# Linux-cpp-lisp/sitator

Measured on AMD Instinct MI355X. Metric: landmark-vectors/sec (frames x mobile atoms), fill + site assignment, higher is better.
Workload: dtype f64; 1 GPU; C2: SCgrid(8,8,8) orthorhombic 32.0x35.2x38.4 A, S=D=512 (V=8), M=64, A=576 (BASELINE configs[1]), 100000 frames per GPU; frames_per_gpu=100000, n_mobile=64, n_static=512, landmark_dim=512, parallelism=frame-sharded x1

## Files before the change

### sitator_amd/csrc/cluster.hip

```cpp
#include <cmath>
#include <cstring>
#include <hip/amd_detail/amd_hip_unsafe_atomics.h>

#include <algorithm>

#include "sit_internal.h"

__device__ __forceinline__ Best wave_best(Best b)
{
    for (int off = 32; off > 0; off >>= 1) {
        Best o;
        o.v = __shfl_down(b.v, off);
        o.i = __shfl_down(b.i, off);
        o.nan = __shfl_down(b.nan, off);
        b = best_merge(b, o);
    }
    return b;
}

#define PRED_BLOCK 256
#define PRED_MAXCOL 24

struct PredArgs {
    const i32 *row_nnz, *row_idx;
    const double *row_val;
    const i32 *col_ptr, *col_k;
    const double *col_val;
    const double *dense;
    i64 *labels;
    double *confs;
    i64 N, K, D;
    int normed;
    double threshold;
};

__device__ __forceinline__ i64 finish_predict(const PredArgs &a, i64 row, Best b)
{
    i64 to; double conf;
    finish_assignment(b, a.threshold, to, conf);
    __builtin_nontemporal_store(to, &a.labels[row]);
    __builtin_nontemporal_store(conf, &a.confs[row]);
    return to;
}

__device__ i64 predict_row_generic(const PredArgs &a, i64 row, int n, double xn)
{
    Best b = best_empty();
    for (int e = 0; e < n; e++) {
        const i32 d = a.row_idx[(i64)e * a.N + row];
        const i32 lo = a.col_ptr[d], hi = a.col_ptr[d + 1];
        for (i32 q = lo; q < hi; q++) {
            const i32 cid = a.col_k[q];
            const double *crow = a.dense + (i64)cid * a.D;
            bool owner = true;
            for (int e2 = 0; e2 < e; e2++) {
                const double cv = crow[a.row_idx[(i64)e2 * a.N + row]];
                if (cv != 0.0) { owner = false; break; }
            }
            if (!owner) continue;
            double dot = 0.0;
            bool first = true;
            for (int e3 = e; e3 < n; e3++) {
                const double cv = crow[a.row_idx[(i64)e3 * a.N + row]];
                if (cv != 0.0) {
                    const double t = cv * a.row_val[(i64)e3 * a.N + row];
                    dot = first ? t : dot + t;
                    first = false;
                }
            }
            if (a.normed) dot /= xn;
            b = best_merge(b, best_of(fabs(dot), cid));
        }
    }
    return finish_predict(a, row, b);
}

__device__ __forceinline__ i64 predict_row_merge(const PredArgs &a, i64 row, int n, double xn)
{
    i32 d0 = a.row_idx[row], d1 = 0, d2 = 0, d3 = 0;
    double v0 = a.row_val[row], v1 = 0, v2 = 0, v3 = 0;
    if (n > 1) { d1 = a.row_idx[a.N + row]; v1 = a.row_val[a.N + row]; }
    if (n > 2) { d2 = a.row_idx[2 * a.N + row]; v2 = a.row_val[2 * a.N + row]; }
    if (n > 3) { d3 = a.row_idx[3 * a.N + row]; v3 = a.row_val[3 * a.N + row]; }
    return finish_predict(a, row, merge4_row(n, d0, d1, d2, d3, v0, v1, v2, v3, xn, a.normed != 0, a.col_ptr, a.col_k, a.col_val));
}

template <int NW>
__device__ __forceinline__ i64 predict_row_merge_wide(const PredArgs &a, i64 row, int n, double xn)
{
    ArgMaxQ am;
    am.init();
    const i32 none = 0x7fffffff;
    i32 q[NW], e[NW], h[NW];
    double v[NW];
#pragma unroll
    for (int s = 0; s < NW; s++) {
        q[s] = 0; e[s] = 0; h[s] = none; v[s] = 0.0;
        if (s < n) {
            const i32 d = a.row_idx[(i64)s * a.N + row];
            q[s] = a.col_ptr[d]; e[s] = a.col_ptr[d + 1]; v[s] = a.row_val[(i64)s * a.N + row];
            h[s] = q[s] < e[s] ? a.col_k[q[s]] : none;
        }
    }
    while (true) {
        i32 cid = h[0];
#pragma unroll
        for (int s = 1; s < NW; s++) cid = h[s] < cid ? h[s] : cid;
        if (cid == none) break;
        double dot = 0.0;
        bool first = true;
#pragma unroll
        for (int s = 0; s < NW; s++) {
            if (h[s] == cid) {
                const double t = a.col_val[q[s]] * v[s];
                dot = first ? t : dot + t;
                first = false;
                q[s]++;
                h[s] = q[s] < e[s] ? a.col_k[q[s]] : none;
            }
        }
        am.push(dot, cid, xn, a.normed != 0);
    }
    return finish_predict(a, row, am.result(xn, a.normed != 0));
}

__device__ __forceinline__ bool predict_row_head(const PredArgs &a, i64 row, int &n, double &xn)
{
    n = __builtin_nontemporal_load(&a.row_nnz[row]);
    if (n == 0) { __builtin_nontemporal_store((i64)-1, &a.labels[row]); __builtin_nontemporal_store(0.0, &a.confs[row]); return false; }
    double x2 = 0.0;
    for (int e = 0; e < n; e++) { const double v = a.row_val[(i64)e * a.N + row]; x2 += v * v; }
    xn = sqrt(x2);
    return true;
}

__device__ __forceinline__ void list_wide_rows(int n, bool live, i64 row, i32 *seg, unsigned *seg_count, i64 seg_cap, int lane)
{
    list_rows_by_class(live && n > 4 && n <= 8, live && n > 8, row, seg, seg_count, seg_cap, lane);
}

__global__ __launch_bounds__(PRED_BLOCK) void k_predict_rows(PredArgs a, i32 *wide_list, unsigned *wide_count, i64 seg_cap)
{
    i32 *seg = wide_list + (i64)blockIdx.x * seg_cap;
    unsigned *seg_count = wide_count + 2 * blockIdx.x;
    const int lane = threadIdx.x & 63;
    for (i64 r0 = (i64)blockIdx.x * PRED_BLOCK; r0 < a.N; r0 += (i64)gridDim.x * PRED_BLOCK) {
        const i64 row = r0 + threadIdx.x;
        int n = 0;
        double xn = 0.0;
        const bool live = row < a.N && predict_row_head(a, row, n, xn);
        const bool wide = live && n > 4;
        list_wide_rows(n, live, row, seg, seg_count, seg_cap, lane);
        if (live && !wide) predict_row_merge(a, row, n, xn);
    }
}

struct ArgMaxR {
    double ms;
    i32 i;
    __device__ __forceinline__ void init() { ms = 0.0; i = -1; }
    __device__ __forceinline__ void push(double dot, i32 cid, double xn, bool normed)
    {
        bool take = !(fabs(dot) <= fabs(ms));
        const bool clear = fabs(dot) > fabs(ms) * (1.0 + 1e-15);
        if (normed & take & !clear)
            take = dot != dot || fabs(dot) / xn > fabs(ms) / xn;
        take = take & (ms == ms);
        ms = take ? dot : ms;
        i = take ? cid : i;
    }
    __device__ __forceinline__ Best result(double xn, bool normed) const
    {
        Best b;
        const double m = fabs(ms);
        b.i = (i64)i; b.nan = m != m ? 1 : 0;
        b.v = i < 0 ? 0.0 : (normed ? m / xn : m);
        return b;
    }
};
typedef const unsigned __attribute__((address_space(3))) *LdsWords;
struct RecHead { i32 h; double hv; unsigned p; };
#define PRED_REC 12
__device__ __forceinline__ void rec_load(RecHead &c)
{
    LdsWords r = (LdsWords)(uintptr_t)c.p;
    const unsigned r0 = r[0], r1 = r[1], r2 = r[2];
    c.h = (i32)r2;
    c.hv = __hiloint2double((int)r1, (int)r0);
}
__device__ __forceinline__ Best merge4_rec(int n, i32 d0, i32 d1, i32 d2, i32 d3, double v0, double v1, double v2, double v3,
                                           double xn, bool normed, const unsigned *l_off)
{
    ArgMaxR am;
    am.init();
    const i32 none = 0x7fffffff;
    RecHead c0, c1, c2, c3;
    c0.p = l_off[d0]; rec_load(c0);
    c1.h = none; c1.hv = 0.0; c1.p = 0u;
    c2 = c1; c3 = c1;
    if (n > 1) { c1.p = l_off[d1]; rec_load(c1); }
    if (n > 2) { c2.p = l_off[d2]; rec_load(c2); }
    if (n > 3) { c3.p = l_off[d3]; rec_load(c3); }
    while (true) {
        i32 cid = c0.h < c1.h ? c0.h : c1.h;
        const i32 m23 = c2.h < c3.h ? c2.h : c3.h;
        cid = cid < m23 ? cid : m23;
        if (cid == none) break;
        double dot = 0.0;
        if (c0.h == cid) { dot = c0.hv * v0; c0.p += PRED_REC; rec_load(c0); }
        if (c1.h == cid) { dot = dot + c1.hv * v1; c1.p += PRED_REC; rec_load(c1); }
        if (c2.h == cid) { dot = dot + c2.hv * v2; c2.p += PRED_REC; rec_load(c2); }
        if (c3.h == cid) { dot = dot + c3.hv * v3; c3.p += PRED_REC; rec_load(c3); }
        am.push(dot, cid, xn, normed);
    }
    return am.result(xn, normed);
}

#define PRED_REC_BLOCK 1024
__global__ __launch_bounds__(PRED_REC_BLOCK) void k_predict_rows_rec(PredArgs a, const unsigned *recs, int nrec, i32 *wide_list, unsigned *wide_count,
                                                                     i64 seg_cap, int hist_K, u64 *counts)
{
    extern __shared__ __attribute__((aligned(16))) char pl_smem[];
    unsigned *l_rec = (unsigned *)pl_smem;
    unsigned *l_off = l_rec + 3 * nrec;
    unsigned *hist = l_off + a.D;
    const int NT = PRED_REC_BLOCK;
    for (int q = threadIdx.x; q < hist_K; q += NT) hist[q] = 0u;
    for (int q = threadIdx.x; q < 3 * nrec; q += NT) l_rec[q] = recs[q];
    for (int q = threadIdx.x; q < (int)a.D; q += NT) l_off[q] = (unsigned)(uintptr_t)(LdsWords)l_rec + (unsigned)PRED_REC * (unsigned)(a.col_ptr[q] + q);
    __syncthreads();
    i32 *seg = wide_list + (i64)blockIdx.x * seg_cap;
    unsigned *seg_count = wide_count + 2 * blockIdx.x;
    const int lane = threadIdx.x & 63;
    for (i64 r0 = (i64)blockIdx.x * NT; r0 < a.N; r0 += (i64)gridDim.x * NT) {
        const i64 row = r0 + threadIdx.x;
        int n = 0;
        double xn = 0.0;
        const bool live = row < a.N && predict_row_head(a, row, n, xn);
        const bool wide = live && n > 4;
        list_wide_rows(n, live, row, seg, seg_count, seg_cap, lane);
        if (live && !wide) {
            i32 d0 = a.row_idx[row], d1 = 0, d2 = 0, d3 = 0;
            double v0 = a.row_val[row], v1 = 0, v2 = 0, v3 = 0;
            if (n > 1) { d1 = a.row_idx[a.N + row]; v1 = a.row_val[a.N + row]; }
            if (n > 2) { d2 = a.row_idx[2 * a.N + row]; v2 = a.row_val[2 * a.N + row]; }
            if (n > 3) { d3 = a.row_idx[3 * a.N + row]; v3 = a.row_val[3 * a.N + row]; }
            const i64 to = finish_predict(a, row, merge4_rec(n, d0, d1, d2, d3, v0, v1, v2, v3, xn, a.normed != 0, l_off));
            if (hist_K > 0 && to >= 0) atomicAdd(&hist[to], 1u);
        }
    }
    if (hist_K > 0) {
        __syncthreads();
        for (int q = threadIdx.x; q < hist_K; q += NT) { const unsigned v = hist[q]; if (v) atomicAdd(&counts[q], (u64)v); }
    }
}

__device__ __forceinline__ void predict_wide_row(const PredArgs &a, i64 row, u64 *counts)
{
    int n;
    double xn;
    if (!predict_row_head(a, row, n, xn)) return;
    i64 to;
    if (n <= 8) to = predict_row_merge_wide<8>(a, row, n, xn);
    else if (n <= 10) to = predict_row_merge_wide<10>(a, row, n, xn);
    else if (n <= 16) to = predict_row_merge_wide<16>(a, row, n, xn);
    else to = predict_row_generic(a, row, n, xn);
    if (counts && to >= 0) atomicAdd(&counts[to], 1ull);
}

__global__ __launch_bounds__(PRED_BLOCK) void k_predict_rows_wide(PredArgs a, const i32 *wide_list, const unsigned *wide_count, i64 seg_cap,
                                                                  int nseg, u64 *counts)
{
    for (int sg = blockIdx.x; sg < nseg; sg += gridDim.x) {
        const i64 na = (i64)wide_count[2 * sg], nb = (i64)wide_count[2 * sg + 1];
        const i32 *seg = wide_list + (i64)sg * seg_cap;
        for (i64 q = threadIdx.x; q < na; q += PRED_BLOCK) predict_wide_row(a, seg[q], counts);
        for (i64 q = threadIdx.x; q < nb; q += PRED_BLOCK) predict_wide_row(a, seg[seg_cap - 1 - q], counts);
    }
}

#define PRED_WIDE_LDS_BLOCK 1024
template <int NW>
__device__ __forceinline__ i64 predict_row_merge_wide_rec(const PredArgs &a, i64 row, int n, double xn, const unsigned *l_off)
{
    ArgMaxR am;
    am.init();
    const i32 none = 0x7fffffff;
    RecHead c[NW];
    double v[NW];
#pragma unroll
    for (int s = 0; s < NW; s++) {
        c[s].h = none; c[s].hv = 0.0; c[s].p = 0u; v[s] = 0.0;
        if (s < n) {
            c[s].p = l_off[a.row_idx[(i64)s * a.N + row]];
            v[s] = a.row_val[(i64)s * a.N + row];
            rec_load(c[s]);
        }
    }
    while (true) {
        i32 cid = c[0].h;
#pragma unroll
        for (int s = 1; s < NW; s++) cid = c[s].h < cid ? c[s].h : cid;
        if (cid == none) break;
        double dot = 0.0;
#pragma unroll
        for (int s = 0; s < NW; s++) {
            if (c[s].h == cid) {
                dot = dot + c[s].hv * v[s];
                c[s].p += PRED_REC;
                rec_load(c[s]);
            }
        }
        am.push(dot, cid, xn, a.normed != 0);
    }
    return finish_predict(a, row, am.result(xn, a.normed != 0));
}

__device__ __forceinline__ void predict_wide_row_rec(const PredArgs &a, i64 row, const unsigned *l_off, u64 *counts)
{
    int n;
    double xn;
    if (!predict_row_head(a, row, n, xn)) return;
    i64 to;
    if (n <= 8) to = predict_row_merge_wide_rec<8>(a, row, n, xn, l_off);
    else if (n <= 10) to = predict_row_merge_wide_rec<10>(a, row, n, xn, l_off);
    else if (n <= 16) to = predict_row_merge_wide_rec<16>(a, row, n, xn, l_off);
    else to = predict_row_generic(a, row, n, xn);
    if (counts && to >= 0) atomicAdd(&counts[to], 1ull);
}

__global__ __launch_bounds__(PRED_WIDE_LDS_BLOCK) void k_predict_rows_wide_rec(PredArgs a, const unsigned *recs, int nrec, const i32 *wide_list,
                                                                              const unsigned *wide_count, i64 seg_cap, int nseg, u64 *counts)
{
    extern __shared__ __attribute__((aligned(16))) char pl_smem[];
    __shared__ unsigned any;
    unsigned *l_rec = (unsigned *)pl_smem;
    unsigned *l_off = l_rec + 3 * nrec;
    if (threadIdx.x == 0) any = 0u;
    __syncthreads();
    for (int sg = blockIdx.x + threadIdx.x * gridDim.x; sg < nseg; sg += gridDim.x * PRED_WIDE_LDS_BLOCK)
        if (wide_count[2 * sg] | wide_count[2 * sg + 1]) any = 1u;
    __syncthreads();
    if (!any) return;
    for (int q = threadIdx.x; q < 3 * nrec; q += PRED_WIDE_LDS_BLOCK) l_rec[q] = recs[q];
    for (int q = threadIdx.x; q < (int)a.D; q += PRED_WIDE_LDS_BLOCK) l_off[q] = (unsigned)(uintptr_t)(LdsWords)l_rec + (unsigned)PRED_REC * (unsigned)(a.col_ptr[q] + q);
    __syncthreads();
    for (int sg = blockIdx.x; sg < nseg; sg += gridDim.x) {
        const i64 na = (i64)wide_count[2 * sg], nb = (i64)wide_count[2 * sg + 1];
        const i32 *seg = wide_list + (i64)sg * seg_cap;
        for (i64 q = threadIdx.x; q < na; q += PRED_WIDE_LDS_BLOCK) predict_wide_row_rec(a, seg[q], l_off, counts);
        for (i64 q = threadIdx.x; q < nb; q += PRED_WIDE_LDS_BLOCK) predict_wide_row_rec(a, seg[seg_cap - 1 - q], l_off, counts);
    }
}

__global__ __launch_bounds__(PRED_BLOCK) void k_predict_rows_dense(PredArgs a)
{
    const i64 row = (i64)blockIdx.x * PRED_BLOCK + threadIdx.x;
    if (row >= a.N) return;
    const int n = a.row_nnz[row];
    if (n == 0) { a.labels[row] = -1; a.confs[row] = 0.0; return; }
    double x2 = 0.0;
    for (int e = 0; e < n; e++) { const double v = a.row_val[(i64)e * a.N + row]; x2 += v * v; }
    const double xn = sqrt(x2);
    Best b = best_empty();
    for (i64 k = 0; k < a.K; k++) {
        double dot = 0.0;
        for (int e = 0; e < n; e++)
            dot += a.dense[k * a.D + a.row_idx[(i64)e * a.N + row]] * a.row_val[(i64)e * a.N + row];
        if (a.normed) dot /= xn;
        b = best_merge(b, best_of(fabs(dot), k));
    }
    (void)finish_predict(a, row, b);
}

extern "C" int sit_set_centers(sit_ctx *c, const double *centers, i64 K, int normed)
{
    if (!c || !centers) return SIT_ERR_INVALID;
    SIT_REQUIRE(c, c->D > 0 && K > 0, "sit_set_centers: basis must be set and K > 0");
    HIP_TRY(c, hipSetDevice(c->device));
    if (c->fill_ring) { const int rcd = fill_results_wait(c); if (rcd) return rcd; }
    const i64 D = c->D;
    std::vector<i32> ptr((size_t)D + 1, 0);
    for (i64 k = 0; k < K; k++) {
        const double *row = centers + k * D;
        for (i64 d = 0; d < D; d++) ptr[(size_t)d + 1] += row[d] != 0.0;
    }
    for (i64 d = 0; d < D; d++) ptr[(size_t)d + 1] += ptr[(size_t)d];
    std::vector<i32> ks((size_t)ptr[(size_t)D]), cur(ptr.begin(), ptr.end() - 1);
    std::vector<double> vals((size_t)ptr[(size_t)D]);
    for (i64 k = 0; k < K; k++) {
        const double *row = centers + k * D;
        for (i64 d = 0; d < D; d++)
            if (row[d] != 0.0) { const i32 q = cur[(size_t)d]++; ks[(size_t)q] = (i32)k; vals[(size_t)q] = row[d]; }
    }
    if (ks.empty()) { ks.push_back(0); vals.push_back(0.0); }
    int rc;
    if ((rc = dev_upload(c, &c->d_col_ptr, ptr.data(), D + 1))) return rc;
    if ((rc = dev_upload(c, &c->d_col_k, ks.data(), (i64)ks.size()))) return rc;
    if ((rc = dev_upload(c, &c->d_col_val, vals.data(), (i64)vals.size()))) return rc;
    {
        const size_t nrec = (size_t)ptr[(size_t)D] + (size_t)D;
        std::vector<unsigned> recs(3 * nrec);
        for (i64 d = 0; d < D; d++) {
            for (i32 q = ptr[(size_t)d]; q < ptr[(size_t)d + 1]; q++) {
                unsigned w[2];
                memcpy(w, &vals[(size_t)q], 8);
                unsigned *r = &recs[3 * ((size_t)q + (size_t)d)];
                r[0] = w[0]; r[1] = w[1]; r[2] = (unsigned)ks[(size_t)q];
            }
            unsigned *e = &recs[3 * ((size_t)ptr[(size_t)d + 1] + (size_t)d)];
            e[0] = 0u; e[1] = 0u; e[2] = 0x7fffffffu;
        }
        if ((rc = dev_upload(c, &c->d_col_rec, recs.data(), (i64)recs.size()))) return rc;
        c->csc_nrec = (i64)nrec;
    }
    c->K = K; c->centers_normed = normed;
    c->csc_nnz = (i64)vals.size();
    c->max_col = 0;
    for (i64 d = 0; d < D; d++) if (ptr[(size_t)d + 1] - ptr[(size_t)d] > c->max_col) c->max_col = ptr[(size_t)d + 1] - ptr[(size_t)d];
    if ((rc = dev_alloc(c, &c->d_counts, K))) return rc;
    if ((rc = dev_upload(c, &c->d_cen_dense, centers, K * D))) return rc;
    c->assign_valid = false;
    return SIT_OK;
}

struct PredPlan {
    bool narrow_lds, wide_lds;
    size_t lds, wide_lds_bytes;
    int nt, per_cu, nseg;
    i64 seg_cap;
    unsigned *wcount;
    i32 *wlist;
};

static void predict_form(const sit_ctx *c, PredPlan &p)
{
    const char *pl = getenv("SITATOR_PREDICT_LDS");
    const bool lds = !(pl && pl[0] == '0') && c->d_col_rec;
    p.wide_lds_bytes = (size_t)c->csc_nrec * PRED_REC + (size_t)c->D * 4;
    p.lds = p.wide_lds_bytes + (size_t)c->K * 4;
    p.narrow_lds = lds && p.lds <= 150 * 1024;
    p.wide_lds = lds && p.wide_lds_bytes <= 150 * 1024;
}

int wide_list_carve(sit_ctx *c, int nseg, i64 seg_cap, unsigned **wcount, i32 **wlist)
{
    const int rc = ensure_scratch(c, ((i64)nseg * seg_cap + 2 * nseg + 64) * 4);
    if (rc) return rc;
    *wcount = (unsigned *)c->d_scratch;
    *wlist = (i32 *)c->d_scratch + ((2 * nseg + 63) / 64 * 64);
    return SIT_OK;
}

static int predict_plan(sit_ctx *c, PredPlan &p)
{
    predict_form(c, p);
    p.nt = p.narrow_lds ? PRED_REC_BLOCK : PRED_BLOCK;
    p.per_cu = !p.narrow_lds ? 8 : (p.lds <= 78 * 1024 ? 2 : 1);
    const i64 blocks = (c->N + p.nt - 1) / p.nt;
    p.nseg = (int)std::min<i64>(blocks, (i64)cu_count(c) * p.per_cu);
    p.seg_cap = (blocks + p.nseg - 1) / p.nseg * p.nt;
    return wide_list_carve(c, p.nseg, p.seg_cap, &p.wcount, &p.wlist);
}

int predict_reset_with_fill(sit_ctx *c, bool *done)
{
    *done = false;
    if (c->N <= 0 || c->K <= 0 || c->max_col > PRED_MAXCOL) return reset_fill_words(c);
    PredPlan pp;
    int rc = predict_plan(c, pp);
    if (rc) return rc;
    if ((rc = reset_step_words(c, pp.narrow_lds, pp.wcount, 2 * pp.nseg))) return rc;
    *done = true;
    return SIT_OK;
}

static int launch_wide_rows(sit_ctx *c, const PredArgs &a, const PredPlan &p, u64 *cnt)
{
    const int ncu = cu_count(c);
    if (p.wide_lds) {
        HIP_TRY(c, lds_limit((const void *)k_predict_rows_wide_rec, p.wide_lds_bytes, c->device));
        k_predict_rows_wide_rec<<<dim3((unsigned)std::min(ncu, p.nseg)), dim3(PRED_WIDE_LDS_BLOCK), p.wide_lds_bytes, c->stream>>>(
            a, c->d_col_rec, (int)c->csc_nrec, p.wlist, p.wcount, p.seg_cap, p.nseg, cnt);
    } else
        k_predict_rows_wide<<<dim3((unsigned)std::min(p.nseg, ncu * 8)), dim3(PRED_BLOCK), 0, c->stream>>>(a, p.wlist, p.wcount, p.seg_cap, p.nseg, cnt);
    return SIT_OK;
}

static int run_predict(sit_ctx *c, double threshold, bool words_reset = false)
{
    SIT_REQUIRE(c, c->rows_valid, "predict: no landmark rows on the device (run sit_fill with store_rows)");
    SIT_REQUIRE(c, c->K > 0 && c->d_col_ptr, "predict: no centres set");
    int rc;
    if (!c->d_labels || c->assign_N != c->N) {
        if ((rc = dev_alloc(c, &c->d_labels, c->N))) return rc;
        if ((rc = dev_alloc(c, &c->d_confs, c->N))) return rc;
        c->assign_N = c->N;
    }
    if (c->N == 0) {
        HIP_TRY(c, hipMemsetAsync(c->d_counts, 0, sizeof(i64) * (size_t)c->K, c->stream));
        c->assign_valid = true;
        return SIT_OK;
    }
    PredArgs a;
    a.row_nnz = c->d_row_nnz; a.row_idx = c->d_row_idx; a.row_val = c->d_row_val;
    a.col_ptr = c->d_col_ptr; a.col_k = c->d_col_k; a.col_val = c->d_col_val; a.dense = c->d_cen_dense;
    a.labels = c->d_labels; a.confs = c->d_confs;
    a.N = c->rows_N; a.K = c->K; a.D = c->D; a.normed = c->centers_normed; a.threshold = threshold;
    SIT_REQUIRE(c, c->N < (1LL << 31), "sit_predict: more than 2^31 rows per context (the wide-row list holds 32-bit row numbers)");
    const unsigned grid = (unsigned)((c->N + PRED_BLOCK - 1) / PRED_BLOCK);
    StageTimer t(c, T_PREDICT);
    bool counted = false;
    if (c->max_col <= PRED_MAXCOL) {
        PredPlan pp;
        if ((rc = predict_plan(c, pp))) return rc;
        if (getenv("SITATOR_DEBUG_SHAPE")) fprintf(stderr, "predict: lds %zu nt %d per_cu %d nseg %d seg_cap %lld narrow_lds %d wide_lds %d rows_W %lld\n", pp.lds, pp.nt, pp.per_cu, pp.nseg, (long long)pp.seg_cap, (int)pp.narrow_lds, (int)pp.wide_lds, (long long)c->rows_W);
        if (!words_reset && (rc = reset_predict_words(c, pp.narrow_lds, pp.wcount, 2 * pp.nseg))) return rc;
        if (pp.narrow_lds) {
            HIP_TRY(c, lds_limit((const void *)k_predict_rows_rec, pp.lds, c->device));
            k_predict_rows_rec<<<dim3((unsigned)pp.nseg), dim3(PRED_REC_BLOCK), pp.lds, c->stream>>>(a, c->d_col_rec, (int)c->csc_nrec, pp.wlist, pp.wcount, pp.seg_cap, (int)c->K, (u64 *)c->d_counts);
            counted = true;
        } else
            k_predict_rows<<<dim3((unsigned)pp.nseg), dim3(PRED_BLOCK), 0, c->stream>>>(a, pp.wlist, pp.wcount, pp.seg_cap);
        if (c->rows_W > 4 && (rc = launch_wide_rows(c, a, pp, counted ? (u64 *)c->d_counts : nullptr))) return rc;
    } else k_predict_rows_dense<<<dim3(grid), dim3(PRED_BLOCK), 0, c->stream>>>(a);
    HIP_TRY(c, hipGetLastError());
    if (!counted && (rc = sit_label_counts(c))) return rc;
    t.stop();
    c->assign_valid = true;
    return SIT_OK;
}

int predict_listed_rows(sit_ctx *c, double threshold, i32 *wlist, unsigned *wcount, i64 seg_cap, int nseg)
{
    PredArgs a;
    a.row_nnz = c->d_row_nnz; a.row_idx = c->d_row_idx; a.row_val = c->d_row_val;
    a.col_ptr = c->d_col_ptr; a.col_k = c->d_col_k; a.col_val = c->d_col_val; a.dense = c->d_cen_dense;
    a.labels = c->d_labels; a.confs = c->d_confs;
    a.N = c->rows_N; a.K = c->K; a.D = c->D; a.normed = c->centers_normed; a.threshold = threshold;
    PredPlan pp;
    predict_form(c, pp);
    pp.nseg = nseg; pp.seg_cap = seg_cap; pp.wcount = wcount; pp.wlist = wlist;
    StageTimer t(c, T_PREDICT);
    { const int rcw = launch_wide_rows(c, a, pp, nullptr); if (rcw) return rcw; }
    HIP_TRY(c, hipGetLastError());
    int rc = sit_label_counts(c, false);
    if (rc) return rc;
    t.stop();
    c->assign_valid = true;
    return SIT_OK;
}

int sit_predict_internal(sit_ctx *c, double threshold, bool words_reset) { return run_predict(c, threshold, words_reset); }

extern "C" int sit_get_assignments(sit_ctx *c, i64 *labels, double *confs, i64 *counts)
{
    if (!c) return SIT_ERR_INVALID;
    SIT_SETTLE(c);
    SIT_REQUIRE(c, c->assign_valid, "no assignments on the device");
    HIP_TRY(c, hipSetDevice(c->device));
    static const size_t staged_min = [] { const char *v = getenv("SITATOR_STAGED_D2H_MB"); const long long n = v ? atoll(v) : -1; return (size_t)(n >= 0 ? n : 64) << 20; }();
    const bool staged = (size_t)c->N * 8 >= staged_min;
    int rc;
    if (labels && c->N) {
        if (staged) { if ((rc = download_staged(c, c->stream, labels, c->d_labels, (size_t)c->N * 8))) return rc; }
        else HIP_TRY(c, hipMemcpyAsync(labels, c->d_labels, (size_t)c->N * 8, hipMemcpyDeviceToHost, c->stream));
    }
    if (confs && c->N) {
        if (staged) { if ((rc = download_staged(c, c->stream, confs, c->d_confs, (size_t)c->N * 8))) return rc; }
        else HIP_TRY(c, hipMemcpyAsync(confs, c->d_confs, (size_t)c->N * 8, hipMemcpyDeviceToHost, c->stream));
    }
    if (counts) HIP_TRY(c, hipMemcpyAsync(counts, c->d_counts, (size_t)c->K * 8, hipMemcpyDeviceToHost, c->stream));
    HIP_TRY(c, hipStreamSynchronize(c->stream));
    return SIT_OK;
}

__global__ __launch_bounds__(256) void k_count_zero_rows(const i32 *nnz, i64 N, u64 *out)
{
    u64 n = 0, first = SIT_NO_ERROR_KEY;
    for (i64 r = (i64)blockIdx.x * 256 + threadIdx.x; r < N; r += (i64)gridDim.x * 256)
        if (nnz[r] == 0) { n++; first = (u64)r < first ? (u64)r : first; }
    for (int off = 32; off > 0; off >>= 1) {
        n += __shfl_down(n, off);
        const u64 o = __shfl_down(first, off);
        first = o < first ? o : first;
    }
    if ((threadIdx.x & 63) == 0 && n) { atomicAdd(&out[0], n); atomicMin(&out[1], first); }
}

extern "C" int sit_count_zero_rows(sit_ctx *c, i64 *n_zero, i64 *first_row)
{
    if (!c || !n_zero || !first_row) return SIT_ERR_INVALID;
    SIT_SETTLE(c);
    SIT_REQUIRE(c, c->rows_valid, "sit_count_zero_rows: no landmark rows on the device");
    HIP_TRY(c, hipSetDevice(c->device));
    HIP_TRY(c, hipMemsetAsync(c->d_scal, 0, sizeof(u64), c->stream));
    HIP_TRY(c, hipMemsetAsync(c->d_scal + 1, 0xFF, sizeof(u64), c->stream));
    if (c->N > 0) {
        const i64 blocks = (c->N + 255) / 256;
        k_count_zero_rows<<<dim3((unsigned)(blocks < 2048 ? blocks : 2048)), dim3(256), 0, c->stream>>>(c->d_row_nnz, c->N, c->d_scal);
        HIP_TRY(c, hipGetLastError());
    }
    u64 *hb = (u64 *)c->h_pinned;
    HIP_TRY(c, hipMemcpyAsync(hb, c->d_scal, 16, hipMemcpyDeviceToHost, c->stream));
    HIP_TRY(c, hipStreamSynchronize(c->stream));
    *n_zero = (i64)hb[0];
    *first_row = hb[0] ? (i64)hb[1] : -1;
    return SIT_OK;
}

extern "C" int sit_predict(sit_ctx *c, double threshold, i64 *labels, double *confs, i64 *counts)
{
    if (!c) return SIT_ERR_INVALID;
    HIP_TRY(c, hipSetDevice(c->device));
    SIT_SETTLE(c);
    int rc = run_predict(c, threshold);
    if (rc) return rc;
    return sit_get_assignments(c, labels, confs, counts);
}

#define FIT_T 512

struct FitArgs {
    const i32 *row_nnz, *row_idx;
    const double *row_val;
    const i64 *weights;
    i64 stride;
    i64 row_begin, row_end;
    i64 D, cap;
    double threshold;
    double *cen, *nrm;
    i64 *cnt, *Kp;
    i64 *status;
};

__global__ __launch_bounds__(FIT_T) void k_fit_stream(FitArgs a)
{
    extern __shared__ __attribute__((aligned(16))) char smem[];
    double *xd = (double *)smem;
    double *ev = xd + a.D;
    i32 *ei = (i32 *)(ev + a.D);
    __shared__ double r_v[FIT_T / 64];
    __shared__ i64 r_i[FIT_T / 64];
    __shared__ int r_n[FIT_T / 64];
    __shared__ double r_s[FIT_T / 64];
    __shared__ i64 sK;
    const int t = threadIdx.x, lane = t & 63, wave = t >> 6;
    for (i64 d = t; d < a.D; d += FIT_T) xd[d] = 0.0;
    if (t == 0) sK = *a.Kp;
    __syncthreads();
    i64 K = sK;
    i64 row = a.row_begin;
    for (; row < a.row_end; row++) {
        const int n = a.row_nnz[row];
        for (int e = t; e < n; e += FIT_T) {
            const i32 d = a.row_idx[(i64)e * a.stride + row];
            const double v = a.row_val[(i64)e * a.stride + row];
            ei[e] = d; ev[e] = v; xd[d] = v;
        }
        __syncthreads();
        const i64 w = a.weights ? a.weights[row] : 1;
        double x2 = 0.0;
        for (int e = 0; e < n; e++) x2 += ev[e] * ev[e];
        const double vn = sqrt(x2);
        i64 to = -1;
        if (K > 0) {
            Best b = best_empty();
            for (i64 k = t; k < K; k += FIT_T) {
                const double *ck = a.cen + k * a.D;
                double dot = 0.0;
                for (int e = 0; e < n; e++) dot += ck[ei[e]] * ev[e];
                dot /= a.nrm[k];
                dot /= vn;
                b = best_merge(b, best_of(dot, k));
            }
            b = wave_best(b);
            if (lane == 0) { r_v[wave] = b.v; r_i[wave] = b.i; r_n[wave] = b.nan; }
            __syncthreads();
            Best g = best_empty();
            for (int q = 0; q < FIT_T / 64; q++) {
                Best o; o.v = r_v[q]; o.i = r_i[q]; o.nan = r_n[q];
                g = best_merge(g, o);
            }
            to = g.i;
            if (g.v < a.threshold) to = -1;
        }
        if (to < 0) {
            if (K == a.cap) break;
            double *ck = a.cen + K * a.D;
            for (i64 d = t; d < a.D; d += FIT_T) ck[d] = xd[d];
            if (t == 0) { a.nrm[K] = vn; a.cnt[K] = w; }
            K++;
            __syncthreads();
        } else {
            double *ck = a.cen + to * a.D;
            const i64 nold = a.cnt[to];
            const double fo = (double)nold, fn = (double)(nold + w);
            double s = 0.0;
            for (i64 d = t; d < a.D; d += FIT_T) {
                double cv = ck[d];
                cv *= fo; cv += xd[d]; cv /= fn;
                ck[d] = cv;
                s += cv * cv;
            }
            for (int off = 32; off > 0; off >>= 1) s += __shfl_down(s, off);
            __syncthreads();
            if (lane == 0) r_s[wave] = s;
            __syncthreads();
            if (t == 0) {
                double tot = 0.0;
                for (int q = 0; q < FIT_T / 64; q++) tot += r_s[q];
                a.nrm[to] = sqrt(tot);
                a.cnt[to] = nold + w;
            }
        }
        for (int e = t; e < n; e += FIT_T) xd[ei[e]] = 0.0;
        __threadfence_block();
        __syncthreads();
    }
    if (t == 0) {
        *a.Kp = K;
        a.status[0] = (row < a.row_end) ? 1 : 0;
        a.status[1] = row;
    }
}

static int fit_ensure(sit_ctx *c, i64 cap)
{
    if (c->fit_cap >= cap && c->d_fit_centers) return SIT_OK;
    double *ncen = nullptr, *nnrm = nullptr;
    i64 *ncnt = nullptr;
    HIP_TRY(c, hipMalloc((void **)&ncen, (size_t)(cap * c->D) * 8));
    HIP_TRY(c, hipMalloc((void **)&nnrm, (size_t)cap * 8));
    HIP_TRY(c, hipMalloc((void **)&ncnt, (size_t)cap * 8));
    if (c->fit_K > 0 && c->d_fit_centers && c->fit_cap > 0) {
        HIP_TRY(c, hipMemcpyAsync(ncen, c->d_fit_centers, (size_t)(c->fit_K * c->D) * 8, hipMemcpyDeviceToDevice, c->stream));
        HIP_TRY(c, hipMemcpyAsync(nnrm, c->d_fit_nrm2, (size_t)c->fit_K * 8, hipMemcpyDeviceToDevice, c->stream));
        HIP_TRY(c, hipMemcpyAsync(ncnt, c->d_fit_counts, (size_t)c->fit_K * 8, hipMemcpyDeviceToDevice, c->stream));
        HIP_TRY(c, hipStreamSynchronize(c->stream));
    }
    if (c->d_fit_centers) (void)hipFree(c->d_fit_centers);
    if (c->d_fit_nrm2) (void)hipFree(c->d_fit_nrm2);
    if (c->d_fit_counts) (void)hipFree(c->d_fit_counts);
    c->d_fit_centers = ncen; c->d_fit_nrm2 = nnrm; c->d_fit_counts = ncnt; c->fit_cap = cap;
    return SIT_OK;
}

extern "C" int sit_fit_reset(sit_ctx *c)
{
    if (!c) return SIT_ERR_INVALID;
    SIT_REQUIRE(c, c->D > 0, "sit_fit_reset: basis must be set");
    HIP_TRY(c, hipSetDevice(c->device));
    c->fit_K = 0;
    HIP_TRY(c, hipMemsetAsync(c->d_fit_K, 0, 8, c->stream));
    int rc = fit_ensure(c, 256);
    if (rc) return rc;
    if (c->fit_use_fast) return fitfast_set_state(c, nullptr, nullptr, 0);
    fitfast_invalidate(c);
    return SIT_OK;
}

__global__ void k_row_norms(const double *cen, i64 K, i64 D, double *nrm)
{
    i64 k = (i64)blockIdx.x * blockDim.x + threadIdx.x;
    if (k >= K) return;
    double s = 0.0;
    for (i64 d = 0; d < D; d++) s += cen[k * D + d] * cen[k * D + d];
    nrm[k] = sqrt(s);
}

extern "C" int sit_fit_set_state(sit_ctx *c, const double *centers, const i64 *counts, i64 K)
{
    if (!c || (K > 0 && (!centers || !counts))) return SIT_ERR_INVALID;
    SIT_REQUIRE(c, c->D > 0, "sit_fit_set_state: basis must be set");
    HIP_TRY(c, hipSetDevice(c->device));
    c->fit_K = 0;
    int rc = fit_ensure(c, K + 256);
    if (rc) return rc;
    if (K > 0) {
        HIP_TRY(c, hipMemcpyAsync(c->d_fit_centers, centers, (size_t)(K * c->D) * 8, hipMemcpyHostToDevice, c->stream));
        HIP_TRY(c, hipMemcpyAsync(c->d_fit_counts, counts, (size_t)K * 8, hipMemcpyHostToDevice, c->stream));
        k_row_norms<<<dim3((unsigned)((K + 63) / 64)), dim3(64), 0, c->stream>>>(c->d_fit_centers, K, c->D, c->d_fit_nrm2);
        HIP_TRY(c, hipGetLastError());
    }
    HIP_TRY(c, hipMemcpyAsync(c->d_fit_K, &K, 8, hipMemcpyHostToDevice, c->stream));
    HIP_TRY(c, hipStreamSynchronize(c->stream));
    c->fit_K = K;
    if (c->fit_use_fast) return fitfast_set_state(c, centers, counts, K);
    fitfast_invalidate(c);
    return SIT_OK;
}

extern "C" int sit_fit_get_state(sit_ctx *c, double *centers, i64 *counts, i64 *K)
{
    if (!c || !K) return SIT_ERR_INVALID;
    HIP_TRY(c, hipSetDevice(c->device));
    if (fitfast_valid(c)) {
        std::vector<double> cen; std::vector<i64> cnt;
        int rc = !centers && !counts ? fitfast_count(c, K) : fitfast_to_dense(c, cen, cnt, K, centers, counts);
        if (rc) return rc;
        c->fit_K = *K;
        return SIT_OK;
    }
    *K = c->fit_K;
    if (c->fit_K > 0) {
        if (centers) HIP_TRY(c, hipMemcpyAsync(centers, c->d_fit_centers, (size_t)(c->fit_K * c->D) * 8, hipMemcpyDeviceToHost, c->stream));
        if (counts) HIP_TRY(c, hipMemcpyAsync(counts, c->d_fit_counts, (size_t)c->fit_K * 8, hipMemcpyDeviceToHost, c->stream));
        HIP_TRY(c, hipStreamSynchronize(c->stream));
    }
    return SIT_OK;
}

static int fit_stream(sit_ctx *c, const i32 *nnz, const i32 *idx, const double *val, const i64 *weights,
                      i64 stride, int width, i64 nrows, double threshold)
{
    int rc;
    i64 begin = 0;
    if (fitfast_valid(c)) {
        if ((rc = fitfast_stream(c, nnz, idx, val, weights, stride, width, nrows, threshold, &begin))) return rc;
        if (getenv("SITATOR_DEBUG_PIPE")) fprintf(stderr, "    fit: step chain took %lld of %lld rows, state %s\n", (long long)begin, (long long)nrows, fitfast_valid(c) ? "valid" : "handed over");
        if (begin >= nrows && fitfast_valid(c)) return SIT_OK;
        std::vector<double> cen; std::vector<i64> cnt; i64 Kd = 0;
        if ((rc = fitfast_to_dense(c, cen, cnt, &Kd))) return rc;
        fitfast_invalidate(c);
        c->fit_K = 0;
        if ((rc = fit_ensure(c, Kd + 256))) return rc;
        if (Kd > 0) {
            HIP_TRY(c, hipMemcpyAsync(c->d_fit_centers, cen.data(), (size_t)(Kd * c->D) * 8, hipMemcpyHostToDevice, c->stream));
            HIP_TRY(c, hipMemcpyAsync(c->d_fit_counts, cnt.data(), (size_t)Kd * 8, hipMemcpyHostToDevice, c->stream));
            k_row_norms<<<dim3((unsigned)((Kd + 63) / 64)), dim3(64), 0, c->stream>>>(c->d_fit_centers, Kd, c->D, c->d_fit_nrm2);
            HIP_TRY(c, hipGetLastError());
        }
        HIP_TRY(c, hipMemcpyAsync(c->d_fit_K, &Kd, 8, hipMemcpyHostToDevice, c->stream));
        HIP_TRY(c, hipStreamSynchronize(c->stream));
        c->fit_K = Kd;
    }
    if (!c->d_fit_centers && (rc = fit_ensure(c, 256))) return rc;
    if ((rc = ensure_scratch(c, 64))) return rc;
    const size_t lds = (size_t)c->D * 20 + 16;
    SIT_REQUIRE(c, lds <= 150 * 1024, "fit: landmark dimension too large for the LDS-resident row");
    HIP_TRY(c, hipFuncSetAttribute((const void *)k_fit_stream, hipFuncAttributeMaxDynamicSharedMemorySize, (int)lds));
    i64 *status = (i64 *)c->d_scal + 4;
// ... 651 lines not shown
```

Baseline: 9.602 billion lvec/s.

## Issue row loads unconditionally and prefetch next rows across LDS staging

```diff
diff --git a/sitator_amd/csrc/cluster.hip b/sitator_amd/csrc/cluster.hip
--- a/sitator_amd/csrc/cluster.hip
+++ b/sitator_amd/csrc/cluster.hip
@@ -31,6 +31,7 @@
     double *confs;
     i64 N, K, D;
     int normed;
+    int W;
     double threshold;
 };
 
@@ -75,30 +76,70 @@
     return finish_predict(a, row, b);
 }
 
-__device__ __forceinline__ i64 predict_row_merge(const PredArgs &a, i64 row, int n, double xn)
-{
-    i32 d0 = a.row_idx[row], d1 = 0, d2 = 0, d3 = 0;
-    double v0 = a.row_val[row], v1 = 0, v2 = 0, v3 = 0;
-    if (n > 1) { d1 = a.row_idx[a.N + row]; v1 = a.row_val[a.N + row]; }
-    if (n > 2) { d2 = a.row_idx[2 * a.N + row]; v2 = a.row_val[2 * a.N + row]; }
-    if (n > 3) { d3 = a.row_idx[3 * a.N + row]; v3 = a.row_val[3 * a.N + row]; }
-    return finish_predict(a, row, merge4_row(n, d0, d1, d2, d3, v0, v1, v2, v3, xn, a.normed != 0, a.col_ptr, a.col_k, a.col_val));
+struct Row4 {
+    int n;
+    i32 d0, d1, d2, d3;
+    double v0, v1, v2, v3;
+};
+__device__ __forceinline__ void row4_request(const PredArgs &a, i64 row, Row4 &r)
+{
+    const i64 rc = row < a.N ? row : a.N - 1;
+    const i64 o1 = a.W > 1 ? a.N : 0, o2 = a.W > 2 ? 2 * a.N : o1, o3 = a.W > 3 ? 3 * a.N : o2;
+    r.n = __builtin_nontemporal_load(&a.row_nnz[rc]);
+    r.d0 = a.row_idx[rc]; r.d1 = a.row_idx[o1 + rc]; r.d2 = a.row_idx[o2 + rc]; r.d3 = a.row_idx[o3 + rc];
+    r.v0 = a.row_val[rc]; r.v1 = a.row_val[o1 + rc]; r.v2 = a.row_val[o2 + rc]; r.v3 = a.row_val[o3 + rc];
+}
+__device__ __forceinline__ void row4_select(const PredArgs &a, i64 row, Row4 &r, double &xn)
+{
+    asm volatile("" : "+v"(r.n), "+v"(r.d0), "+v"(r.d1), "+v"(r.d2), "+v"(r.d3), "+v"(r.v0), "+v"(r.v1), "+v"(r.v2), "+v"(r.v3));
+    const int n = row < a.N ? r.n : 0;
+    r.n = n;
+    r.d0 = n > 0 ? r.d0 : 0; r.v0 = n > 0 ? r.v0 : 0.0;
+    r.d1 = n > 1 ? r.d1 : 0; r.v1 = n > 1 ? r.v1 : 0.0;
+    r.d2 = n > 2 ? r.d2 : 0; r.v2 = n > 2 ? r.v2 : 0.0;
+    r.d3 = n > 3 ? r.d3 : 0; r.v3 = n > 3 ? r.v3 : 0.0;
+    double x2 = 0.0;
+    x2 += r.v0 * r.v0; x2 += r.v1 * r.v1; x2 += r.v2 * r.v2; x2 += r.v3 * r.v3;
+    xn = sqrt(x2);
 }
 
 template <int NW>
-__device__ __forceinline__ i64 predict_row_merge_wide(const PredArgs &a, i64 row, int n, double xn)
+__device__ __forceinline__ void wide_row_load(const PredArgs &a, i64 row, int n, i32 (&d)[NW], double (&v)[NW], double &xn)
+{
+#pragma unroll
+    for (int s = 0; s < NW; s++) d[s] = a.row_idx[(s < n ? (i64)s * a.N : 0) + row];
+#pragma unroll
+    for (int s = 0; s < NW; s++) v[s] = a.row_val[(s < n ? (i64)s * a.N : 0) + row];
+    if (NW > 8) {
+        asm volatile("" : "+v"(d[0]), "+v"(d[1]), "+v"(d[2]), "+v"(d[3]), "+v"(d[4]), "+v"(d[5]), "+v"(d[6]), "+v"(d[7]), "+v"(d[NW - 2]), "+v"(d[NW - 1]),
+                          "+v"(v[NW - 2]), "+v"(v[NW - 1]));
+    } else
+        asm volatile("" : "+v"(d[0]), "+v"(d[NW - 1]), "+v"(v[0]), "+v"(v[NW - 1]));
+    double x2 = 0.0;
+#pragma unroll
+    for (int s = 0; s < NW; s++) {
+        d[s] = s < n ? d[s] : 0;
+        v[s] = s < n ? v[s] : 0.0;
+        x2 += v[s] * v[s];
+    }
+    xn = sqrt(x2);
+}
+
+template <int NW>
+__device__ __forceinline__ i64 predict_row_merge_wide(const PredArgs &a, i64 row, int n)
 {
     ArgMaxQ am;
     am.init();
     const i32 none = 0x7fffffff;
     i32 q[NW], e[NW], h[NW];
-    double v[NW];
+    double v[NW], xn;
+    wide_row_load<NW>(a, row, n, h, v, xn);
 #pragma unroll
     for (int s = 0; s < NW; s++) {
-        q[s] = 0; e[s] = 0; h[s] = none; v[s] = 0.0;
+        const i32 d = h[s];
+        q[s] = 0; e[s] = 0; h[s] = none;
         if (s < n) {
-            const i32 d = a.row_idx[(i64)s * a.N + row];
-            q[s] = a.col_ptr[d]; e[s] = a.col_ptr[d + 1]; v[s] = a.row_val[(i64)s * a.N + row];
+            q[s] = a.col_ptr[d]; e[s] = a.col_ptr[d + 1];
             h[s] = q[s] < e[s] ? a.col_k[q[s]] : none;
         }
     }
@@ -124,13 +165,16 @@
     return finish_predict(a, row, am.result(xn, a.normed != 0));
 }
 
-__device__ __forceinline__ bool predict_row_head(const PredArgs &a, i64 row, int &n, double &xn)
+__device__ __forceinline__ double row_norm(const PredArgs &a, i64 row, int n)
+{
+    double x2 = 0.0;
+    for (int e = 0; e < n; e++) { const double v = a.row_val[(i64)e * a.N + row]; x2 += v * v; }
+    return sqrt(x2);
+}
+__device__ __forceinline__ bool wide_row_count(const PredArgs &a, i64 row, int &n)
 {
     n = __builtin_nontemporal_load(&a.row_nnz[row]);
     if (n == 0) { __builtin_nontemporal_store((i64)-1, &a.labels[row]); __builtin_nontemporal_store(0.0, &a.confs[row]); return false; }
-    double x2 = 0.0;
-    for (int e = 0; e < n; e++) { const double v = a.row_val[(i64)e * a.N + row]; x2 += v * v; }
-    xn = sqrt(x2);
     return true;
 }
 
@@ -146,12 +190,15 @@
     const int lane = threadIdx.x & 63;
     for (i64 r0 = (i64)blockIdx.x * PRED_BLOCK; r0 < a.N; r0 += (i64)gridDim.x * PRED_BLOCK) {
         const i64 row = r0 + threadIdx.x;
-        int n = 0;
-        double xn = 0.0;
-        const bool live = row < a.N && predict_row_head(a, row, n, xn);
-        const bool wide = live && n > 4;
-        list_wide_rows(n, live, row, seg, seg_count, seg_cap, lane);
-        if (live && !wide) predict_row_merge(a, row, n, xn);
+        Row4 r;
+        double xn;
+        row4_request(a, row, r);
+        row4_select(a, row, r, xn);
+        const bool live = r.n != 0, wide = r.n > 4;
+        if (row < a.N && !live) { __builtin_nontemporal_store((i64)-1, &a.labels[row]); __builtin_nontemporal_store(0.0, &a.confs[row]); }
+        list_wide_rows(r.n, live, row, seg, seg_count, seg_cap, lane);
+        if (live && !wide)
+            finish_predict(a, row, merge4_row(r.n, r.d0, r.d1, r.d2, r.d3, r.v0, r.v1, r.v2, r.v3, xn, a.normed != 0, a.col_ptr, a.col_k, a.col_val));
     }
 }
 
@@ -195,12 +242,13 @@
     am.init();
     const i32 none = 0x7fffffff;
     RecHead c0, c1, c2, c3;
-    c0.p = l_off[d0]; rec_load(c0);
-    c1.h = none; c1.hv = 0.0; c1.p = 0u;
-    c2 = c1; c3 = c1;
-    if (n > 1) { c1.p = l_off[d1]; rec_load(c1); }
-    if (n > 2) { c2.p = l_off[d2]; rec_load(c2); }
-    if (n > 3) { c3.p = l_off[d3]; rec_load(c3); }
+    c0.p = l_off[d0]; c1.p = l_off[d1]; c2.p = l_off[d2]; c3.p = l_off[d3];
+    asm volatile("" : "+v"(c0.p), "+v"(c1.p), "+v"(c2.p), "+v"(c3.p));
+    rec_load(c0); rec_load(c1); rec_load(c2); rec_load(c3);
+    asm volatile("" : "+v"(c0.h), "+v"(c1.h), "+v"(c2.h), "+v"(c3.h));
+    if (n <= 1) { c1.h = none; c1.hv = 0.0; }
+    if (n <= 2) { c2.h = none; c2.hv = 0.0; }
+    if (n <= 3) { c3.h = none; c3.hv = 0.0; }
     while (true) {
         i32 cid = c0.h < c1.h ? c0.h : c1.h;
         const i32 m23 = c2.h < c3.h ? c2.h : c3.h;
@@ -216,6 +264,27 @@
     return am.result(xn, normed);
 }
 
+template <int NT>
+__device__ __forceinline__ void stage_columns(unsigned *l_rec, unsigned *l_off, const unsigned *recs, int nrec, const i32 *col_ptr, int D)
+{
+    const int nw = 3 * nrec;
+    for (int q0 = threadIdx.x; q0 - (int)threadIdx.x < nw; q0 += 8 * NT) {
+        unsigned t[8];
+#pragma unroll
+        for (int u = 0; u < 8; u++) { const int q = min(q0 + u * NT, nw - 1); t[u] = recs[q]; }
+#pragma unroll
+        for (int u = 0; u < 8; u++) { const int q = min(q0 + u * NT, nw - 1); l_rec[q] = t[u]; }
+    }
+    const unsigned base = (unsigned)(uintptr_t)(LdsWords)l_rec;
+    for (int q0 = threadIdx.x; q0 - (int)threadIdx.x < D; q0 += 4 * NT) {
+        i32 t[4];
+#pragma unroll
+        for (int u = 0; u < 4; u++) { const int q = min(q0 + u * NT, D - 1); t[u] = col_ptr[q]; }
+#pragma unroll
+        for (int u = 0; u < 4; u++) { const int q = min(q0 + u * NT, D - 1); l_off[q] = base + (unsigned)PRED_REC * (unsigned)(t[u] + q); }
+    }
+}
+
 #define PRED_REC_BLOCK 1024
 __global__ __launch_bounds__(PRED_REC_BLOCK) void k_predict_rows_rec(PredArgs a, const unsigned *recs, int nrec, i32 *wide_list, unsigned *wide_count,
                                                                      i64 seg_cap, int hist_K, u64 *counts)
@@ -225,29 +294,33 @@
     unsigned *l_off = l_rec + 3 * nrec;
     unsigned *hist = l_off + a.D;
     const int NT = PRED_REC_BLOCK;
+    i64 r0 = (i64)blockIdx.x * NT;
+    if (r0 >= a.N) return;
+    Row4 r;
+    row4_request(a, r0 + threadIdx.x, r);
     for (int q = threadIdx.x; q < hist_K; q += NT) hist[q] = 0u;
-    for (int q = threadIdx.x; q < 3 * nrec; q += NT) l_rec[q] = recs[q];
-    for (int q = threadIdx.x; q < (int)a.D; q += NT) l_off[q] = (unsigned)(uintptr_t)(LdsWords)l_rec + (unsigned)PRED_REC * (unsigned)(a.col_ptr[q] + q);
+    stage_columns<NT>(l_rec, l_off, recs, nrec, a.col_ptr, (int)a.D);
     __syncthreads();
     i32 *seg = wide_list + (i64)blockIdx.x * seg_cap;
     unsigned *seg_count = wide_count + 2 * blockIdx.x;
     const int lane = threadIdx.x & 63;
-    for (i64 r0 = (i64)blockIdx.x * NT; r0 < a.N; r0 += (i64)gridDim.x * NT) {
+    while (true) {
         const i64 row = r0 + threadIdx.x;
-        int n = 0;
-        double xn = 0.0;
-        const bool live = row < a.N && predict_row_head(a, row, n, xn);
-        const bool wide = live && n > 4;
-        list_wide_rows(n, live, row, seg, seg_count, seg_cap, lane);
-        if (live && !wide) {
-            i32 d0 = a.row_idx[row], d1 = 0, d2 = 0, d3 = 0;
-            double v0 = a.row_val[row], v1 = 0, v2 = 0, v3 = 0;
-            if (n > 1) { d1 = a.row_idx[a.N + row]; v1 = a.row_val[a.N + row]; }
-            if (n > 2) { d2 = a.row_idx[2 * a.N + row]; v2 = a.row_val[2 * a.N + row]; }
-            if (n > 3) { d3 = a.row_idx[3 * a.N + row]; v3 = a.row_val[3 * a.N + row]; }
-            const i64 to = finish_predict(a, row, merge4_rec(n, d0, d1, d2, d3, v0, v1, v2, v3, xn, a.normed != 0, l_off));
+        double xn;
+        row4_select(a, row, r, xn);
+        list_wide_rows(r.n, r.n != 0, row, seg, seg_count, seg_cap, lane);
+        if (row < a.N && r.n <= 4) {
+            const Best b = merge4_rec(r.n, r.d0, r.d1, r.d2, r.d3, r.v0, r.v1, r.v2, r.v3, xn, a.normed != 0, l_off);
+            i64 to; double conf;
+            finish_assignment(b, a.threshold, to, conf);
+            if (r.n == 0) { to = -1; conf = 0.0; }
+            __builtin_nontemporal_store(to, &a.labels[row]);
+            __builtin_nontemporal_store(conf, &a.confs[row]);
             if (hist_K > 0 && to >= 0) atomicAdd(&hist[to], 1u);
         }
+        r0 += (i64)gridDim.x * NT;
+        if (r0 >= a.N) break;
+        row4_request(a, r0 + threadIdx.x, r);
     }
     if (hist_K > 0) {
         __syncthreads();
@@ -258,13 +331,12 @@
 __device__ __forceinline__ void predict_wide_row(const PredArgs &a, i64 row, u64 *counts)
 {
     int n;
-    double xn;
-    if (!predict_row_head(a, row, n, xn)) return;
+    if (!wide_row_count(a, row, n)) return;
     i64 to;
-    if (n <= 8) to = predict_row_merge_wide<8>(a, row, n, xn);
-    else if (n <= 10) to = predict_row_merge_wide<10>(a, row, n, xn);
-    else if (n <= 16) to = predict_row_merge_wide<16>(a, row, n, xn);
-    else to = predict_row_generic(a, row, n, xn);
+    if (n <= 8) to = predict_row_merge_wide<8>(a, row, n);
+    else if (n <= 10) to = predict_row_merge_wide<10>(a, row, n);
+    else if (n <= 16) to = predict_row_merge_wide<16>(a, row, n);
+    else to = predict_row_generic(a, row, n, row_norm(a, row, n));
     if (counts && to >= 0) atomicAdd(&counts[to], 1ull);
 }
 
@@ -281,22 +353,22 @@
 
 #define PRED_WIDE_LDS_BLOCK 1024
 template <int NW>
-__device__ __forceinline__ i64 predict_row_merge_wide_rec(const PredArgs &a, i64 row, int n, double xn, const unsigned *l_off)
+__device__ __forceinline__ i64 predict_row_merge_wide_rec(const PredArgs &a, i64 row, int n, const unsigned *l_off)
 {
     ArgMaxR am;
     am.init();
     const i32 none = 0x7fffffff;
     RecHead c[NW];
-    double v[NW];
-#pragma unroll
-    for (int s = 0; s < NW; s++) {
-        c[s].h = none; c[s].hv = 0.0; c[s].p = 0u; v[s] = 0.0;
-        if (s < n) {
-            c[s].p = l_off[a.row_idx[(i64)s * a.N + row]];
-            v[s] = a.row_val[(i64)s * a.N + row];
-            rec_load(c[s]);
-        }
-    }
+    i32 d[NW];
+    double v[NW], xn;
+    wide_row_load<NW>(a, row, n, d, v, xn);
+#pragma unroll
+    for (int s = 0; s < NW; s++) c[s].p = l_off[d[s]];
+#pragma unroll
+    for (int s = 0; s < NW; s++) rec_load(c[s]);
+#pragma unroll
+    for (int s = 0; s < NW; s++)
+        if (s >= n) { c[s].h = none; c[s].hv = 0.0; }
     while (true) {
         i32 cid = c[0].h;
 #pragma unroll
@@ -319,13 +391,12 @@
 __device__ __forceinline__ void predict_wide_row_rec(const PredArgs &a, i64 row, const unsigned *l_off, u64 *counts)
 {
     int n;
-    double xn;
-    if (!predict_row_head(a, row, n, xn)) return;
+    if (!wide_row_count(a, row, n)) return;
     i64 to;
-    if (n <= 8) to = predict_row_merge_wide_rec<8>(a, row, n, xn, l_off);
-    else if (n <= 10) to = predict_row_merge_wide_rec<10>(a, row, n, xn, l_off);
-    else if (n <= 16) to = predict_row_merge_wide_rec<16>(a, row, n, xn, l_off);
-    else to = predict_row_generic(a, row, n, xn);
+    if (n <= 8) to = predict_row_merge_wide_rec<8>(a, row, n, l_off);
+    else if (n <= 10) to = predict_row_merge_wide_rec<10>(a, row, n, l_off);
+    else if (n <= 16) to = predict_row_merge_wide_rec<16>(a, row, n, l_off);
+    else to = predict_row_generic(a, row, n, row_norm(a, row, n));
     if (counts && to >= 0) atomicAdd(&counts[to], 1ull);
 }
 
@@ -342,8 +413,7 @@
         if (wide_count[2 * sg] | wide_count[2 * sg + 1]) any = 1u;
     __syncthreads();
     if (!any) return;
-    for (int q = threadIdx.x; q < 3 * nrec; q += PRED_WIDE_LDS_BLOCK) l_rec[q] = recs[q];
-    for (int q = threadIdx.x; q < (int)a.D; q += PRED_WIDE_LDS_BLOCK) l_off[q] = (unsigned)(uintptr_t)(LdsWords)l_rec + (unsigned)PRED_REC * (unsigned)(a.col_ptr[q] + q);
+    stage_columns<PRED_WIDE_LDS_BLOCK>(l_rec, l_off, recs, nrec, a.col_ptr, (int)a.D);
     __syncthreads();
     for (int sg = blockIdx.x; sg < nseg; sg += gridDim.x) {
         const i64 na = (i64)wide_count[2 * sg], nb = (i64)wide_count[2 * sg + 1];
@@ -506,7 +576,7 @@
     a.row_nnz = c->d_row_nnz; a.row_idx = c->d_row_idx; a.row_val = c->d_row_val;
     a.col_ptr = c->d_col_ptr; a.col_k = c->d_col_k; a.col_val = c->d_col_val; a.dense = c->d_cen_dense;
     a.labels = c->d_labels; a.confs = c->d_confs;
-    a.N = c->rows_N; a.K = c->K; a.D = c->D; a.normed = c->centers_normed; a.threshold = threshold;
+    a.N = c->rows_N; a.K = c->K; a.D = c->D; a.normed = c->centers_normed; a.W = (int)c->rows_W; a.threshold = threshold;
     SIT_REQUIRE(c, c->N < (1LL << 31), "sit_predict: more than 2^31 rows per context (the wide-row list holds 32-bit row numbers)");
     const unsigned grid = (unsigned)((c->N + PRED_BLOCK - 1) / PRED_BLOCK);
     StageTimer t(c, T_PREDICT);
@@ -537,7 +607,7 @@
     a.row_nnz = c->d_row_nnz; a.row_idx = c->d_row_idx; a.row_val = c->d_row_val;
     a.col_ptr = c->d_col_ptr; a.col_k = c->d_col_k; a.col_val = c->d_col_val; a.dense = c->d_cen_dense;
     a.labels = c->d_labels; a.confs = c->d_confs;
-    a.N = c->rows_N; a.K = c->K; a.D = c->D; a.normed = c->centers_normed; a.threshold = threshold;
+    a.N = c->rows_N; a.K = c->K; a.D = c->D; a.normed = c->centers_normed; a.W = (int)c->rows_W; a.threshold = threshold;
     PredPlan pp;
     predict_form(c, pp);
     pp.nseg = nseg; pp.seg_cap = seg_cap; pp.wcount = wcount; pp.wlist = wlist;
```

Result: no change. 9.564 billion lvec/s (-0.4%).
